# microsoft/protnote

Hardware: AMD Instinct MI355X
Metric: protein-label pairs/sec (fwd+bwd) (higher is better)
Workload: dtype f32

## Files before the change

### protnote_amd/csrc/abi_heads_eval.hpp

```cpp
extern "C" size_t pn_mlp_rows_ws_bytes(const pn_mlp* m, int rows) {
  size_t b = 0;
  int hmax = 0;
  for (int i = 0; i + 1 < m->nlayers; ++i) hmax = m->dims[i + 1] > hmax ? m->dims[i + 1] : hmax;
  b += 2 * al256((size_t)rows * hmax * sizeof(float));
  b += 2 * al256((size_t)hmax * sizeof(float));
  return b;
}

extern "C" int pn_mlp_rows_fwd_eval(const pn_mlp* m, const float* x, int ldx, int rows, float* y, void* ws,
                                    size_t ws_bytes, void* stream) {
  PN_OK(math_field_check(m->math_mode, "pn_mlp_rows_fwd_eval"));
  MathScope math_scope(m->math_mode);
  hipStream_t st = (hipStream_t)stream;
  if (m->nlayers < 1 || m->nlayers > PN_MAX_LAYERS) return fail("mlp: bad layer count %d", m->nlayers);
  for (int i = 0; i <= m->nlayers; ++i)
    if (i < m->nlayers && m->dims[i] % 4 != 0) return fail("mlp: dims[%d]=%d not a multiple of 4", i, m->dims[i]);
  if (ldx % 4 != 0) return fail("mlp: ldx %% 4 != 0");
  int hmax = 0;
  for (int i = 0; i + 1 < m->nlayers; ++i) hmax = m->dims[i + 1] > hmax ? m->dims[i + 1] : hmax;
  Bump bp(ws, ws_bytes);
  float* buf[2];
  buf[0] = bp.take<float>((size_t)rows * hmax);
  buf[1] = bp.take<float>((size_t)rows * hmax);
  float* s = bp.take<float>(hmax);
// ... 439 lines not shown
    if (part == nullptr) return fail("gemm_tn: no partial buffer");
    p.Cpart = part;
    p.ldc = p.N;
    long rps = (p.R + ns - 1) / ns;
    p.rows_per_split = (rps + 31) / 32 * 32;
    ns = (int)((p.R + p.rows_per_split - 1) / p.rows_per_split);
  }
  const unsigned tiles = (unsigned)((p.M / 256) * (p.N / 256));
  dim3 grid(tiles, (unsigned)ns);
  p.task_ns = 0;
  int* sync_ws = p.task_sync;
  p.task_sync = nullptr;
  if (p.M == 3072 && p.N == 3072 && ns >= 2) {
    p.task_ns = ns;
    grid = dim3(tn_task_grid(ns), 1);
    if (SYNC && sync_ws != nullptr && ns * 4 * 4 <= TN_SYNC_INTS) {
      HIP_OK(hipMemsetAsync(sync_ws, 0, (size_t)ns * 4 * 4 * sizeof(int), st));
      p.task_sync = sync_ws;
    }
  }
  {
    ProfScope ps(100 + TA_PLAIN * 10 + TB, 2.0 * (double)R_all * (double)p.M * (double)p.N, st);
    hipLaunchKernelGGL(kern, grid, dim3(512), TN_FAST_LDS_BYTES, st, p);
    if (tail != 0) {
      auto tk = gemm_tn_kernel<TA_PLAIN, TB, false>;
      static bool tattr[64] = {false};
      if (dev < 64 && !tattr[dev]) {
        HIP_OK(hipFuncSetAttribute((const void*)tk, hipFuncAttributeMaxDynamicSharedMemorySize, TN_LDS_BYTES));
        tattr[dev] = true;
      }
      TnParams t = p;
      t.R = R_all; t.row_base = R_all - tail; t.rows_per_split = 32;
      t.Cpart = part + (size_t)ns * p.M * p.N; t.ldc = p.N; t.task_ns = 0; t.task_sync = nullptr;
      hipLaunchKernelGGL(tk, dim3((unsigned)((p.M / 128) * (p.N / 128)), 1), dim3(256), TN_LDS_BYTES, st, t);
    }
  }
  HIP_OK(hipGetLastError());
  if (ns > 1 || tail != 0) {
    hipLaunchKernelGGL(k_splitk_reduce, dim3(nblk((long)p.M * p.N, 256)), dim3(256), 0, st, (const float*)part,
                       ns + (tail != 0 ? 1 : 0), p.M, p.N, (long)p.N, dst, ldd);
    HIP_OK(hipGetLastError());
  }
  return 0;
}

template <int TB, int NP = 3, bool TR = false, bool ABF16 = false>
static int launch_tn_bf16x3(TnParams p, float* dst, long ldd, float* part, size_t part_cap_floats, hipStream_t st) {
  void (*kern)(TnParams) = nullptr;
  constexpr bool SYNC = TR && TB == TB_AFFINE_RELU;
  void (*kern_alt)(TnParams) = nullptr;
  if constexpr (TR) {
    kern = gemm_tn_bf16tr_kernel<TB, ABF16, SYNC, true>;
    kern_alt = gemm_tn_bf16tr_kernel<TB, ABF16, SYNC, false>;
  } else {
    kern = gemm_tn_bf16x3_kernel<TB, NP>;
  }
  constexpr int LDS = TR ? TN_BF16TR_LDS_BYTES : 2 * 512 * 36 * (int)sizeof(float);
  static std::atomic<bool> attr_done[64];
  int dev = 0;
  HIP_OK(hipGetDevice(&dev));
  if (dev < 64 && !attr_done[dev]) {
    HIP_OK(hipFuncSetAttribute((const void*)kern, hipFuncAttributeMaxDynamicSharedMemorySize, LDS));
    if (kern_alt != nullptr) HIP_OK(hipFuncSetAttribute((const void*)kern_alt, hipFuncAttributeMaxDynamicSharedMemorySize, LDS));
    attr_done[dev] = true;
  }
  if (kern_alt != nullptr && !g_bf16_m16.load()) kern = kern_alt;
  int ns = tn_pick_split(p.R, p.M, p.N, part_cap_floats, 256, 1);
  if (ns == 1) {
    p.Cpart = dst;
    p.ldc = ldd;
    p.rows_per_split = (p.R + 31) / 32 * 32;
  } else {
    if (part == nullptr) return fail("gemm_tn: no partial buffer");
    p.Cpart = part;
    p.ldc = p.N;
    long rps = (p.R + ns - 1) / ns;
    p.rows_per_split = (rps + 31) / 32 * 32;
    ns = (int)((p.R + p.rows_per_split - 1) / p.rows_per_split);
  }
  const unsigned tiles = (unsigned)((p.M / 256) * (p.N / 256));
  dim3 grid(tiles, (unsigned)ns);
  p.task_ns = 0;
  int* sync_ws = p.task_sync;
  p.task_sync = nullptr;
  if (p.M == 3072 && p.N == 3072 && ns >= 2) {
    p.task_ns = ns;
    grid = dim3(tn_task_grid(ns), 1);
    if (SYNC && sync_ws != nullptr && ns * 4 * 4 <= TN_SYNC_INTS) {
      HIP_OK(hipMemsetAsync(sync_ws, 0, (size_t)ns * 4 * 4 * sizeof(int), st));
      p.task_sync = sync_ws;
    }
  }
  {
    ProfScope ps((NP == 3 ? 1100 : 1600) + TB, 2.0 * (double)p.R * (double)p.M * (double)p.N, st);
    hipLaunchKernelGGL(kern, grid, dim3(512), LDS, st, p);
  }
  HIP_OK(hipGetLastError());
  if (ns > 1) {
    hipLaunchKernelGGL(k_splitk_reduce, dim3(nblk((long)p.M * p.N, 256)), dim3(256), 0, st, (const float*)part, ns,
                       p.M, p.N, (long)p.N, dst, ldd);
    HIP_OK(hipGetLastError());
  }
  return 0;
}

template <int TA, int TB>
// ... 72 lines not shown
```

### protnote_amd/csrc/gemm_bf16x3.hpp

```cpp
#pragma once
#include "gemm_engine.hpp"
#include "gemm_tn.hpp"

#ifndef PN_B3_VALU
#define PN_B3_VALU 4
#endif

namespace pn {

typedef __bf16 bf16x4 __attribute__((ext_vector_type(4)));
typedef __bf16 bf16x8 __attribute__((ext_vector_type(8)));
typedef float f32x4 __attribute__((ext_vector_type(4)));

struct HiLo {
  bf16x4 hi, lo;
};

typedef __bf16 bf16x2 __attribute__((ext_vector_type(2)));
typedef float f32x2 __attribute__((ext_vector_type(2)));

__device__ __forceinline__ void split2(float x0, float x1, uint32_t& hi, uint32_t& lo) {
  const f32x2 x = {x0, x1};
  const bf16x2 h = __builtin_convertvector(x, bf16x2);
  hi = __builtin_bit_cast(uint32_t, h);
  const float r0 = x0 - __uint_as_float(hi << 16);
  const float r1 = x1 - __uint_as_float(hi & 0xffff0000u);
  const f32x2 r = {r0, r1};
  lo = __builtin_bit_cast(uint32_t, __builtin_convertvector(r, bf16x2));
}

__device__ __forceinline__ HiLo split4(float4 v) {
  uint32_t h0, l0, h1, l1;
  split2(v.x, v.y, h0, l0);
  split2(v.z, v.w, h1, l1);
  typedef uint32_t u32x2 __attribute__((ext_vector_type(2)));
  HiLo r;
  r.hi = __builtin_bit_cast(bf16x4, (u32x2){h0, h1});
  r.lo = __builtin_bit_cast(bf16x4, (u32x2){l0, l1});
  return r;
}

__device__ __forceinline__ bf16x8 round8(float4 v0, float4 v1) {
  typedef float f32x8 __attribute__((ext_vector_type(8)));
  const f32x8 x = {v0.x, v0.y, v0.z, v0.w, v1.x, v1.y, v1.z, v1.w};
  return __builtin_convertvector(x, bf16x8);
}

template <int AK, int EK, int WAVES_M, int WAVES_N, int WM, int WN, bool GEN = false, bool BDMA = false, int NP = 3>
__global__ __launch_bounds__(WAVES_M* WAVES_N * 64, (WAVES_M * WAVES_N) / 4) void gemm_nt_bf16x3_kernel(const GemmParams p) {
  static_assert(!BDMA || (!GEN && WAVES_M * WAVES_N == 8 && WAVES_N * WN * 32 == 256), "BDMA: 256-column pair-grid tiles");
  static_assert(NP == 3 || (NP == 1 && BDMA), "the single-product variant is built for the DMA-staged pair-grid kernel");
  constexpr int BK = 32;
  constexpr int NT = WAVES_M * WAVES_N * 64;
  constexpr int BM = WAVES_M * WM * 32;
  constexpr int BN = WAVES_N * WN * 32;
  constexpr int LDK = BK + 4;
  constexpr int KV = BK / 8;
  constexpr int RPP = NT / KV;
  constexpr int NQA = BM / RPP;
  constexpr int NQB = (BN + RPP - 1) / RPP;
  static_assert(BM % RPP == 0, "tile/thread mismatch");
  static_assert(AK == A_PLAIN || AK == A_AFFINE_RELU || AK == A_PAIRSUM_RELU || AK == A_CONV,
                "operand kind not built for bf16x3");
  static_assert(AK != A_CONV || GEN, "the conv gather needs the general path");
  constexpr int BPLANE = BN * 16;
  constexpr int STAGE = BDMA ? BM * LDK + 2 * BPLANE : (BM + BN) * LDK;

  extern __shared__ __attribute__((aligned(16))) float smem[];

  const int tid = threadIdx.x;
  const int lane = tid & 63;
  const int wave = tid >> 6;
  const int wm = wave / WAVES_N;
  const int wn = wave % WAVES_N;

  int tile_m, tile_n;
  if (!tile_coords<BM, BN>(p, tile_m, tile_n)) return;
  const int row0 = tile_m * BM;
  const int col0 = tile_n * BN;

  constexpr int NDQ = NP == 3 ? 4 : 2;
  const uint16_t* bsrc[4] = {nullptr, nullptr, nullptr, nullptr};
  unsigned bdst[4] = {0, 0, 0, 0};
  if constexpr (BDMA) {
    const int w = __builtin_amdgcn_readfirstlane(wave);
#pragma unroll
    for (int q = 0; q < NDQ; ++q) {
      const int c = NDQ * w + q;
      const int r = 16 * (c & 15) + (lane >> 2);
      const int g = (lane & 3) ^ ((r >> 2) & 3);
      bsrc[q] = ((c >> 4) ? p.w_lo : p.w_hi) + (long)(col0 + r) * p.Kseg + 8 * g;
      bdst[q] = (unsigned)(BM * LDK + (c >> 4) * BPLANE + 16 * (c & 15) * 16) * 4u;
    }
  }
  const unsigned lds0_b = (unsigned)(uintptr_t)(const __attribute__((address_space(3))) float*)smem;
  auto issue_b_dma = [&](int s_, int buf) {
#pragma unroll
    for (int q = 0; q < NDQ; ++q)
      tn_glds16(reinterpret_cast<const float*>(bsrc[q] + s_ * BK),
                __builtin_amdgcn_readfirstlane(lds0_b + (unsigned)(buf * STAGE) * 4u + bdst[q]));
  };

// ... 56 lines not shown
        for (int h = 0; h < 2; ++h) {
          rsc[h] = ld4(p.a_scale + c + 4 * kv + 16 * h);
          rsh[h] = ld4(p.a_shift + c + 4 * kv + 16 * h);
        }
      }
    } else {
      const int seg = s / spt;
      const int c0 = (s - seg * spt) * BK;
      bool kok[2];
      int cc[2];
#pragma unroll
      for (int h = 0; h < 2; ++h) {
        kok[h] = c0 + 4 * kv + 16 * h < p.Kseg;
        cc[h] = kok[h] ? c0 + 16 * h : -4 * kv;
      }
      avalid = 0;
      if constexpr (AK == A_CONV) {
        const int sh = (seg - p.nseg / 2) * p.dil;
#pragma unroll
        for (int q = 0; q < NQA; ++q) {
          const int tt = a_t[q] + sh;
          const bool ok = (a_t[q] < a_len[q]) && (tt >= 0) && (tt < a_len[q]);
#pragma unroll
          for (int h = 0; h < 2; ++h) {
            ra[q][h] = ld4(arow[q] + (long)(ok ? sh : 0) * p.lda + cc[h]);
            avalid |= ((ok && kok[h]) ? 1u : 0u) << (2 * q + h);
          }
        }
      } else {
#pragma unroll
        for (int q = 0; q < NQA; ++q)
#pragma unroll
          for (int h = 0; h < 2; ++h) {
            ra[q][h] = ld4(arow[q] + cc[h]);
            if constexpr (AK == A_PAIRSUM_RELU) ra2[q][h] = ld4(arow2[q] + cc[h]);
            avalid |= (kok[h] ? 1u : 0u) << (2 * q + h);
          }
      }
      if (AK == A_AFFINE_RELU || conv_affine) {
#pragma unroll
        for (int h = 0; h < 2; ++h) {
          rsc[h] = ld4(p.a_scale + 4 * kv + cc[h]);
          rsh[h] = ld4(p.a_shift + 4 * kv + cc[h]);
        }
      }
    }
  };
  auto fetch_b = [&](int s) {
    if constexpr (!GEN) {
      const int c = s * BK;
#pragma unroll
      for (int q = 0; q < NQB; ++q)
#pragma unroll
        for (int h = 0; h < 2; ++h) rb[q][h] = ld4(brow[q] + c + 16 * h);
    } else {
      const int seg = s / spt;
      const int c0 = (s - seg * spt) * BK;
      bmask = 0;
#pragma unroll
      for (int h = 0; h < 2; ++h) {
        const bool kok = c0 + 4 * kv + 16 * h < p.Kseg;
        const int cc = kok ? c0 + 16 * h : -4 * kv;
#pragma unroll
        for (int q = 0; q < NQB; ++q) {
          rb[q][h] = ld4(brow[q] + (long)seg * p.Kseg + cc);
          bmask |= ((kok && bvalid[q]) ? 1u : 0u) << (2 * q + h);
        }
      }
    }
  };
  auto pin_a = [&]() {
#pragma unroll
    for (int q = 0; q < NQA; ++q)
#pragma unroll
      for (int h = 0; h < 2; ++h) {
        pin4(ra[q][h]);
        if constexpr (AK == A_PAIRSUM_RELU) pin4(ra2[q][h]);
      }
  };
  auto pin_b = [&]() {
#pragma unroll
    for (int q = 0; q < NQB; ++q)
#pragma unroll
      for (int h = 0; h < 2; ++h) pin4(rb[q][h]);
  };

  auto store8 = [](float* dst, float4 v0, float4 v1) {
    if constexpr (NP == 1) {
      *reinterpret_cast<bf16x8*>(dst) = round8(v0, v1);
      return;
    }
    const HiLo a = split4(v0), b = split4(v1);
    bf16x8 hi, lo;
#pragma unroll
    for (int e = 0; e < 4; ++e) {
      hi[e] = a.hi[e];
      hi[4 + e] = b.hi[e];
      lo[e] = a.lo[e];
      lo[4 + e] = b.lo[e];
    }
    *reinterpret_cast<bf16x8*>(dst) = hi;
    *reinterpret_cast<bf16x8*>(dst + 4) = lo;
  };

  auto sel4 = [](bool ok, float4 v) {
    return make_float4(ok ? v.x : 0.f, ok ? v.y : 0.f, ok ? v.z : 0.f, ok ? v.w : 0.f);
  };
  auto commit_a = [&](int buf) {
    float* As = smem + buf * STAGE;
#pragma unroll
    for (int q = 0; q < NQA; ++q) {
      float4 v[2];
#pragma unroll
      for (int h = 0; h < 2; ++h) {
        v[h] = ra[q][h];
        if (AK == A_AFFINE_RELU || (AK == A_CONV && conv_affine)) {
          v[h].x = relu(fmaf(v[h].x, rsc[h].x, rsh[h].x));
          v[h].y = relu(fmaf(v[h].y, rsc[h].y, rsh[h].y));
          v[h].z = relu(fmaf(v[h].z, rsc[h].z, rsh[h].z));
          v[h].w = relu(fmaf(v[h].w, rsc[h].w, rsh[h].w));
        } else if constexpr (AK == A_PAIRSUM_RELU) {
          v[h].x = relu(v[h].x + ra2[q][h].x);
          v[h].y = relu(v[h].y + ra2[q][h].y);
          v[h].z = relu(v[h].z + ra2[q][h].z);
          v[h].w = relu(v[h].w + ra2[q][h].w);
        }
        if constexpr (GEN) v[h] = sel4((avalid >> (2 * q + h)) & 1u, v[h]);
      }
      store8(As + (r_in + q * RPP) * LDK + 8 * kv, v[0], v[1]);
    }
  };
  auto commit_b = [&](int buf) {
    float* Bs = smem + buf * STAGE + BM * LDK;
#pragma unroll
    for (int q = 0; q < NQB; ++q) {
      float4 v0 = rb[q][0], v1 = rb[q][1];
      if constexpr (GEN) {
        v0 = sel4((bmask >> (2 * q)) & 1u, v0);
        v1 = sel4((bmask >> (2 * q + 1)) & 1u, v1);
      }
      if (BN % RPP == 0 || r_in + q * RPP < BN) store8(Bs + (r_in + q * RPP) * LDK + 8 * kv, v0, v1);
    }
  };

  f32x16 acc[WM][WN];
#pragma unroll
  for (int i = 0; i < WM; ++i)
#pragma unroll
    for (int j = 0; j < WN; ++j)
#pragma unroll
      for (int e = 0; e < 16; ++e) acc[i][j][e] = 0.f;

  const int frag_row = lane & 31;
  const int frag_g = lane >> 5;

  auto compute = [&](int buf, auto ks_c) {
    constexpr int KS = decltype(ks_c)::value;
    const float* As = smem + buf * STAGE + (wm * WM * 32 + frag_row) * LDK + (2 * KS + frag_g) * 8;
    bf16x8 ah[WM], al[WM], bh[WN], bl[WN];
#pragma unroll
    for (int i = 0; i < WM; ++i) {
      ah[i] = *reinterpret_cast<const bf16x8*>(As + i * 32 * LDK);
      if constexpr (NP == 3) al[i] = *reinterpret_cast<const bf16x8*>(As + i * 32 * LDK + 4);
    }
    if constexpr (BDMA) {
      const float* Bs = smem + buf * STAGE + BM * LDK + (wn * WN * 32 + frag_row) * 16 +
                        4 * ((2 * KS + frag_g) ^ ((frag_row >> 2) & 3));
#pragma unroll
      for (int j = 0; j < WN; ++j) {
        bh[j] = *reinterpret_cast<const bf16x8*>(Bs + j * 32 * 16);
        if constexpr (NP == 3) bl[j] = *reinterpret_cast<const bf16x8*>(Bs + j * 32 * 16 + BPLANE);
      }
    } else {
      const float* Bs = smem + buf * STAGE + BM * LDK + (wn * WN * 32 + frag_row) * LDK + (2 * KS + frag_g) * 8;
#pragma unroll
      for (int j = 0; j < WN; ++j) {
        bh[j] = *reinterpret_cast<const bf16x8*>(Bs + j * 32 * LDK);
        bl[j] = *reinterpret_cast<const bf16x8*>(Bs + j * 32 * LDK + 4);
      }
    }
#pragma unroll
    for (int i = 0; i < WM; ++i)
#pragma unroll
      for (int j = 0; j < WN; ++j) {
        if constexpr (NP == 3) {
          acc[i][j] = __builtin_amdgcn_mfma_f32_32x32x16_bf16(al[i], bh[j], acc[i][j], 0, 0, 0);
          acc[i][j] = __builtin_amdgcn_mfma_f32_32x32x16_bf16(ah[i], bl[j], acc[i][j], 0, 0, 0);
        }
        acc[i][j] = __builtin_amdgcn_mfma_f32_32x32x16_bf16(ah[i], bh[j], acc[i][j], 0, 0, 0);
      }
  };

  using std::integral_constant;
  auto weave = [&](auto nvalu_c) {
    constexpr int NV = decltype(nvalu_c)::value;
    if constexpr (NP == 1) {
      __builtin_amdgcn_sched_group_barrier(0x100, WM + WN, 0);
#pragma unroll
      for (int i = 0; i < WM * WN; ++i) {
        __builtin_amdgcn_sched_group_barrier(0x008, 1, 0);
        __builtin_amdgcn_sched_group_barrier(0x002, NV, 0);
        if (i % 4 == 3) __builtin_amdgcn_sched_group_barrier(0x200, 1, 0);
      }
      return;
    }
    __builtin_amdgcn_sched_group_barrier(0x100, 2 * (WM + WN), 0);
#pragma unroll
    for (int i = 0; i < WM * WN * 3; ++i) {
      __builtin_amdgcn_sched_group_barrier(0x008, 1, 0);
      __builtin_amdgcn_sched_group_barrier(0x002, NV, 0);
      if (i % 3 == 2) __builtin_amdgcn_sched_group_barrier(0x200, 1, 0);
    }
  };
  if constexpr (BDMA) {
    issue_b_dma(0, 0);
    fetch_a(0);
    pin_a();
    commit_a(0);
    fetch_a(nslab > 1 ? 1 : 0);
    asm volatile("s_waitcnt vmcnt(0) lgkmcnt(0)" ::: "memory");
    __builtin_amdgcn_s_barrier();
    for (int s = 0; s + 1 < nslab; ++s) {
      const int cur = s & 1;
      const int nxt = s + 2 < nslab ? s + 2 : s + 1;
      __builtin_amdgcn_sched_barrier(0);
      pin_a();
      issue_b_dma(s + 1, cur ^ 1);
      __builtin_amdgcn_sched_barrier(0);
      compute(cur, integral_constant<int, 0>{});
      commit_a(cur ^ 1);
      weave(integral_constant<int, (AK == A_PLAIN ? PN_B3_VALU : PN_B3_VALU + 1)>{});
      __builtin_amdgcn_sched_barrier(0);
      asm volatile("s_waitcnt vmcnt(0)" ::: "memory");
      fetch_a(nxt);
      __builtin_amdgcn_sched_barrier(0);
      compute(cur, integral_constant<int, 1>{});
      __builtin_amdgcn_sched_barrier(0);
      asm volatile("s_waitcnt lgkmcnt(0)" ::: "memory");
      __builtin_amdgcn_s_barrier();
    }
    compute((nslab - 1) & 1, integral_constant<int, 0>{});
    __builtin_amdgcn_sched_barrier(0);
    compute((nslab - 1) & 1, integral_constant<int, 1>{});
    __syncthreads();
  } else {
  fetch_a(0);
  fetch_b(0);
  pin_a();
  pin_b();
  commit_a(0);
  commit_b(0);
  fetch_a(nslab > 1 ? 1 : 0);
  fetch_b(nslab > 1 ? 1 : 0);
  __syncthreads();
  for (int s = 0; s + 1 < nslab; ++s) {
    const int cur = s & 1;
    const int nxt = s + 2 < nslab ? s + 2 : s + 1;
    __builtin_amdgcn_sched_barrier(0);
    pin_a();
    compute(cur, integral_constant<int, 0>{});
    commit_a(cur ^ 1);
    weave(integral_constant<int, (AK == A_PLAIN ? PN_B3_VALU : PN_B3_VALU + 1)>{});
    __builtin_amdgcn_sched_barrier(0);
    fetch_a(nxt);
    __builtin_amdgcn_sched_barrier(0);
    pin_b();
    compute(cur, integral_constant<int, 1>{});
    commit_b(cur ^ 1);
    weave(integral_constant<int, PN_B3_VALU>{});
    __builtin_amdgcn_sched_barrier(0);
    fetch_b(nxt);
    __syncthreads();
  }
  compute((nslab - 1) & 1, integral_constant<int, 0>{});
  __builtin_amdgcn_sched_barrier(0);
  compute((nslab - 1) & 1, integral_constant<int, 1>{});
  __syncthreads();
  }

  gemm_epilogue<EK, WAVES_M, WAVES_N, WM, WN>(p, acc, row0, col0, tile_n, smem);
}

template <int TB, int NP = 3>
__global__ __launch_bounds__(512, PN_MINW) void gemm_tn_bf16x3_kernel(const TnParams p) {
  constexpr int BM = 256, BN = 256, BK = 32, LDK = BK + 4;
  constexpr int WM = 2, WN = 4;
  constexpr int STAGE = (BM + BN) * LDK;
  static_assert(TB == TB_PLAIN || TB == TB_AFFINE_RELU || TB == TB_PAIRSUM_RELU, "operand kind not built for bf16x3");

  extern __shared__ __attribute__((aligned(16))) float smem[];

  const int tid = threadIdx.x;
  const int lane = tid & 63;
  const int wave = tid >> 6;
  const int wm = wave >> 1, wn = wave & 1;

  const int ntn = p.N / BN, ntm = p.M / BM;
  int tile_m, tile_n;
  int split = blockIdx.y;
  if (p.task_ns > 0) {
    if (!tn_task_coords(p.task_ns, tile_m, tile_n, split)) return;
  } else if (PN_XCD && TB == TB_PAIRSUM_RELU && (ntm % 4 == 0) && (ntn % 2 == 0)) {
    const int rm = ntm / 4, rn = ntn / 2;
    const int xcd = blockIdx.x & 7, w = blockIdx.x >> 3;
    tile_m = (xcd >> 1) * rm + w / rn;
    tile_n = (xcd & 1) * rn + w % rn;
  } else if (PN_XCD && (ntm % 2 == 0) && (ntn % 4 == 0)) {
    const int rm = ntm / 2, rn = ntn / 4;
    const int xcd = blockIdx.x & 7, w = blockIdx.x >> 3;
    tile_m = (xcd >> 2) * rm + w / rn;
    tile_n = (xcd & 3) * rn + w % rn;
  } else {
    tile_n = blockIdx.x % ntn;
    tile_m = blockIdx.x / ntn;
  }
  const int m0 = tile_m * BM, n0 = tile_n * BN;
  const long r_begin = (long)split * p.rows_per_split;
  long r_end = r_begin + p.rows_per_split;
  if (r_end > p.R) r_end = p.R;

  const int col = tid & 255;
  const int kg = __builtin_amdgcn_readfirstlane(tid >> 8);
  float bs = 0.f, bt = 0.f;
  if constexpr (TB == TB_AFFINE_RELU) {
    bs = p.b_s[n0 + col];
    bt = p.b_t[n0 + col];
  }

  float ra[2][8], rb[2][8], rb2[2];
  const unsigned pB = (unsigned)p.pairB;
  const long lda = p.lda, ldb = p.ldb;

  auto fetch_a = [&](long k0, auto safe_c) {
    constexpr bool SAFE = decltype(safe_c)::value;
    const float* Ak = p.A + k0 * lda + m0;
    const int lim = (int)(r_end - 1 - k0);
#pragma unroll
// ... 56 lines not shown
      if constexpr (TB == TB_PAIRSUM_RELU) asm volatile("" : "+v"(rb2[g]));
    }
  };

  auto store8 = [](float* dst, const float (&v)[8]) {
    if constexpr (NP == 1) {
      *reinterpret_cast<bf16x8*>(dst) = round8(make_float4(v[0], v[1], v[2], v[3]), make_float4(v[4], v[5], v[6], v[7]));
      return;
    }
    const HiLo a = split4(make_float4(v[0], v[1], v[2], v[3])), b = split4(make_float4(v[4], v[5], v[6], v[7]));
    bf16x8 hi, lo;
#pragma unroll
    for (int e = 0; e < 4; ++e) {
      hi[e] = a.hi[e];
      hi[4 + e] = b.hi[e];
      lo[e] = a.lo[e];
      lo[4 + e] = b.lo[e];
    }
    *reinterpret_cast<bf16x8*>(dst) = hi;
    *reinterpret_cast<bf16x8*>(dst + 4) = lo;
  };

  auto commit_a = [&](int buf, long k0, auto safe_c) {
    constexpr bool SAFE = decltype(safe_c)::value;
    float* As = smem + buf * STAGE;
#pragma unroll
    for (int g = 0; g < 2; ++g) {
      float a[8];
#pragma unroll
      for (int e = 0; e < 8; ++e) {
        a[e] = ra[g][e];
        if (SAFE && k0 + 8 * (kg + 2 * g) + e >= r_end) a[e] = 0.f;
      }
      store8(As + col * LDK + 8 * (kg + 2 * g), a);
    }
  };
  auto commit_b = [&](int buf, long k0, auto safe_c) {
    constexpr bool SAFE = decltype(safe_c)::value;
    float* Bs = smem + buf * STAGE + BM * LDK;
#pragma unroll
    for (int g = 0; g < 2; ++g) {
      float b[8];
#pragma unroll
      for (int e = 0; e < 8; ++e) {
        b[e] = rb[g][e];
        if constexpr (TB == TB_AFFINE_RELU) b[e] = relu(fmaf(b[e], bs, bt));
        if constexpr (TB == TB_PAIRSUM_RELU) b[e] = relu(b[e] + rb2[g]);
        if (SAFE && k0 + 8 * (kg + 2 * g) + e >= r_end) b[e] = 0.f;
      }
      store8(Bs + col * LDK + 8 * (kg + 2 * g), b);
    }
  };

  f32x16 acc[WM][WN];
#pragma unroll
  for (int i = 0; i < WM; ++i)
#pragma unroll
    for (int j = 0; j < WN; ++j)
#pragma unroll
      for (int e = 0; e < 16; ++e) acc[i][j][e] = 0.f;

  const int frag_row = lane & 31;
  const int frag_g = lane >> 5;
  auto compute = [&](int buf, auto ks_c) {
    constexpr int KS = decltype(ks_c)::value;
    const float* As = smem + buf * STAGE + (wm * WM * 32 + frag_row) * LDK + (2 * KS + frag_g) * 8;
    const float* Bs = smem + buf * STAGE + BM * LDK + (wn * WN * 32 + frag_row) * LDK + (2 * KS + frag_g) * 8;
    bf16x8 ah[WM], al[WM], bh[WN], bl[WN];
#pragma unroll
    for (int i = 0; i < WM; ++i) {
      ah[i] = *reinterpret_cast<const bf16x8*>(As + i * 32 * LDK);
      if constexpr (NP == 3) al[i] = *reinterpret_cast<const bf16x8*>(As + i * 32 * LDK + 4);
    }
#pragma unroll
    for (int j = 0; j < WN; ++j) {
      bh[j] = *reinterpret_cast<const bf16x8*>(Bs + j * 32 * LDK);
      if constexpr (NP == 3) bl[j] = *reinterpret_cast<const bf16x8*>(Bs + j * 32 * LDK + 4);
    }
#pragma unroll
    for (int i = 0; i < WM; ++i)
#pragma unroll
      for (int j = 0; j < WN; ++j) {
        if constexpr (NP == 3) {
          acc[i][j] = __builtin_amdgcn_mfma_f32_32x32x16_bf16(al[i], bh[j], acc[i][j], 0, 0, 0);
          acc[i][j] = __builtin_amdgcn_mfma_f32_32x32x16_bf16(ah[i], bl[j], acc[i][j], 0, 0, 0);
        }
        acc[i][j] = __builtin_amdgcn_mfma_f32_32x32x16_bf16(ah[i], bh[j], acc[i][j], 0, 0, 0);
      }
  };

  using std::integral_constant;
  using std::false_type;
  using std::true_type;
  auto weave = [&](auto nvalu_c) {
    constexpr int NV = decltype(nvalu_c)::value;
    if constexpr (NP == 1) {
      __builtin_amdgcn_sched_group_barrier(0x100, WM + WN, 0);
#pragma unroll
      for (int i = 0; i < WM * WN; ++i) {
        __builtin_amdgcn_sched_group_barrier(0x008, 1, 0);
        __builtin_amdgcn_sched_group_barrier(0x002, 3 * NV, 0);
        if (i % 4 == 3) __builtin_amdgcn_sched_group_barrier(0x200, 1, 0);
      }
      return;
    }
    __builtin_amdgcn_sched_group_barrier(0x100, 2 * (WM + WN), 0);
#pragma unroll
    for (int i = 0; i < WM * WN * 3; ++i) {
      __builtin_amdgcn_sched_group_barrier(0x008, 1, 0);
      __builtin_amdgcn_sched_group_barrier(0x002, NV, 0);
      if (i % 3 == 2) __builtin_amdgcn_sched_group_barrier(0x200, 1, 0);
    }
  };
  if (r_begin < r_end) {
    const long span = r_end - r_begin;
    const int nf = (int)(span / BK);
    const int ns = nf + ((span % BK) ? 1 : 0);
    auto K0 = [&](int t) { return r_begin + (long)t * BK; };
    auto body = [&](int t, auto safe_c) {
      const int cur = t & 1;
      const int t2 = t + 2 < ns ? t + 2 : t + 1;
      __builtin_amdgcn_sched_barrier(0);
      pin_a();
      compute(cur, integral_constant<int, 0>{});
      commit_a(cur ^ 1, K0(t + 1), safe_c);
      weave(integral_constant<int, 2>{});
      __builtin_amdgcn_sched_barrier(0);
      fetch_a(K0(t2), safe_c);
      __builtin_amdgcn_sched_barrier(0);
      pin_b();
      compute(cur, integral_constant<int, 1>{});
      commit_b(cur ^ 1, K0(t + 1), safe_c);
      weave(integral_constant<int, (TB == TB_PLAIN ? 2 : 3)>{});
      __builtin_amdgcn_sched_barrier(0);
      fetch_b(K0(t2), safe_c);
      __syncthreads();
    };
    fetch_a(K0(0), true_type{});
    fetch_b(K0(0), true_type{});
    pin_a();
    pin_b();
    commit_a(0, K0(0), true_type{});
    commit_b(0, K0(0), true_type{});
    fetch_a(K0(ns > 1 ? 1 : 0), true_type{});
    fetch_b(K0(ns > 1 ? 1 : 0), true_type{});
    __syncthreads();
    int t = 0;
    for (; t + 2 < nf; ++t) body(t, false_type{});
    for (; t + 1 < ns; ++t) body(t, true_type{});
    compute((ns - 1) & 1, integral_constant<int, 0>{});
    __builtin_amdgcn_sched_barrier(0);
    compute((ns - 1) & 1, integral_constant<int, 1>{});
  }

  float* out = p.Cpart + (long)split * p.M * p.ldc;
  const int hl = lane >> 5, cl = lane & 31;
#pragma unroll
  for (int i = 0; i < WM; ++i)
#pragma unroll
    for (int j = 0; j < WN; ++j) {
      const int n = n0 + (wn * WN + j) * 32 + cl;
#pragma unroll
      for (int e = 0; e < 16; ++e) {
        const int m = m0 + (wm * WM + i) * 32 + (e & 3) + 8 * (e >> 2) + 4 * hl;
        out[(long)m * p.ldc + n] = acc[i][j][e];
      }
    }
}

__global__ void k_split_planes(const float* __restrict__ W, long ldw, int N, int K, uint16_t* __restrict__ hi,
                               uint16_t* __restrict__ lo) {
  const long i = ((long)blockIdx.x * blockDim.x + threadIdx.x) * 4;
  if (i >= (long)N * K) return;
  const long n = i / K;
  const int pos = (int)(i - n * K);
  const int blk = pos >> 5, in = pos & 31, g = in >> 3, half = (in >> 2) & 1;
  const HiLo s = split4(ld4(W + n * ldw + blk * 32 + half * 16 + 4 * g));
  *reinterpret_cast<bf16x4*>(hi + i) = s.hi;
  *reinterpret_cast<bf16x4*>(lo + i) = s.lo;
}

}
```

### protnote_amd/csrc/protnote_hip.hip

```cpp
#include <hip/hip_runtime.h>
#include <stdarg.h>
#include <stdio.h>
#include <stdlib.h>
#include <string.h>

#include "../../include/protnote_hip.h"
#include "common.hpp"
#include "gemm_engine.hpp"
#include "gemm_bf16x3.hpp"
#include "gemm_bf16.hpp"
#include "gemm_dma.hpp"
#include "gemm_conv_dma.hpp"
#include "gemm_conv_f64.hpp"
#include "gemm_tn_fast.hpp"
#include "train_kernels.hpp"
#include "bwd_bf16_dz.hpp"
#include "fwd_bf16_h.hpp"
#include "gemm_bf16_m16.hpp"

using namespace pn;

static thread_local char g_err[512] = "";

static int fail(const char* fmt, ...) {
// ... 302 lines not shown
  return 0;
}

static std::atomic<int> g_bwd_math{0};
extern "C" int pn_set_backward_math(int mode) {
  if (mode != 0 && mode != 1) return fail("pn_set_backward_math: 0 (as the forward) or 1 (bf16, one product)");
  g_bwd_math = mode;
  return 0;
}
extern "C" int pn_get_backward_math(void) { return g_bwd_math; }
static thread_local bool tl_bwd_bf16 = false;
static thread_local bool tl_dz_bf16 = false;
struct BwdBf16Scope {
  bool prev;
  explicit BwdBf16Scope(bool on) : prev(tl_bwd_bf16) { tl_bwd_bf16 = on; }
  ~BwdBf16Scope() {
    tl_bwd_bf16 = prev;
    tl_dz_bf16 = false;
  }
};

static std::atomic<int> g_fwd_math{0};
extern "C" int pn_set_forward_math(int mode) {
  if (mode != 0 && mode != 1) return fail("pn_set_forward_math: 0 (as math_mode) or 1 (bf16, one product)");
  g_fwd_math = mode;
  return 0;
}
extern "C" int pn_get_forward_math(void) { return g_fwd_math; }
static thread_local bool tl_fwd_bf16 = false;
struct FwdBf16Scope {
  bool prev;
  explicit FwdBf16Scope(bool on) : prev(tl_fwd_bf16) { tl_fwd_bf16 = on; }
  ~FwdBf16Scope() { tl_fwd_bf16 = prev; }
};
static bool fwd_bf16_requested(const pn_pairhead* hd) {
  const int m = hd->forward_math == 0 ? g_fwd_math.load(std::memory_order_relaxed) : hd->forward_math - 1;
  return m == 1 && hd->dropout_p == 0.f;
}
static int fwd_math_of(const pn_pairhead* hd, bool* bf16) {
  if (hd->forward_math < 0 || hd->forward_math > 2)
    return fail("pairhead: forward_math %d (0 = library default, 1 = as math_mode, 2 = bf16)", hd->forward_math);
  const int m = hd->forward_math == 0 ? g_fwd_math.load(std::memory_order_relaxed) : hd->forward_math - 1;
  *bf16 = (m == 1) && hd->dropout_p == 0.f;
  return 0;
}

static std::atomic<int> g_b3_dma{1};
static bool use_b3_dma() { return g_b3_dma == 1; }
extern "C" int pn_set_b3_dma(int on) {
  g_b3_dma = on ? 1 : 0;
  return 0;
}

template <int AK, int EK, int WAVES_N, int WN, bool GEN, bool BDMA = false, int NP = 3>
static int launch_gemm_bf16x3(const GemmParams& p, hipStream_t st) {
  using Cfg = GemmCfg<4, WAVES_N, 2, WN, 32>;
  if constexpr (!GEN && !BDMA && WAVES_N * WN * 32 == 256) {
    if (p.wsplit != nullptr && use_b3_dma() && p.Nstore == p.N)
      return launch_gemm_bf16x3<AK, EK, WAVES_N, WN, GEN, true>(p, st);
  }
  auto kern = gemm_nt_bf16x3_kernel<AK, EK, 4, WAVES_N, 2, WN, GEN, BDMA, NP>;
  constexpr int LDS_BYTES = BDMA ? 2 * (256 * 36 + 2 * 256 * 16) * (int)sizeof(float) : Cfg::LDS_BYTES;
  static std::atomic<bool> attr_done[64];
  int dev = 0;
  HIP_OK(hipGetDevice(&dev));
  if (dev < 64 && !attr_done[dev]) {
    HIP_OK(hipFuncSetAttribute((const void*)kern, hipFuncAttributeMaxDynamicSharedMemorySize, LDS_BYTES));
    attr_done[dev] = true;
  }
  if (p.M <= 0 || p.Nstore <= 0) return 0;
  if (p.Kseg % 4 != 0) return fail("gemm: K segment %d not a multiple of 4", p.Kseg);
  const long tm = (p.M + Cfg::BM - 1) / Cfg::BM;
  const long tn = (p.Nstore + Cfg::BN - 1) / Cfg::BN;
  GemmParams pp = p;
  pp.xcd_bc = (PN_XCD && tm >= 16) ? ((tn % 8 == 0) ? 8 : ((tn % 4 == 0) ? 4 : 0)) : 0;
  if (!GEN && AK == A_PAIRSUM_RELU && pp.xcd_bc && tm >= 64) pp.xcd_bc = 1;
  pp.xcd_br = pp.xcd_bc ? 32 / pp.xcd_bc : 0;
  long grid = tm * tn;
  if (pp.xcd_bc) {
    const long nblk = ((tm + pp.xcd_br - 1) / pp.xcd_br) * (tn / pp.xcd_bc);
    grid = ((nblk + 7) / 8) * 8 * 32;
  }
  if (grid > 0x7fffffffL) return fail("gemm: grid too large");
  if constexpr (BDMA) {
    pp.w_hi = p.wsplit;
    pp.w_lo = p.wsplit + (size_t)p.N * p.Kseg;
    hipLaunchKernelGGL(k_split_planes, dim3(nblk((long)p.N * p.Kseg / 4, 256)), dim3(256), 0, st, p.W, p.ldw, p.N, p.Kseg,
                       p.wsplit, p.wsplit + (size_t)p.N * p.Kseg);
  }
  {
    ProfScope ps((NP == 3 ? 1000 : 1500) + AK * 10 + EK, 2.0 * (double)p.M * (double)p.N * (double)p.nseg * (double)p.Kseg, st);
    hipLaunchKernelGGL(kern, dim3((unsigned)grid), dim3(Cfg::NT), LDS_BYTES, st, pp);
  }
  HIP_OK(hipGetLastError());
  return finish_col_stats(p, tm, st);
}

static std::atomic<int> g_bwd_deep{7};
extern "C" int pn_set_bwd_deep(int mask) {
  g_bwd_deep = mask & 7;
  return 0;
}
static int launch_gemm_bf16_single(const GemmParams& p, hipStream_t st) {
  auto kern = gemm_nt_bf16_kernel<E_STORE>;
  static std::atomic<bool> attr_done[64];
  int dev = 0;
  HIP_OK(hipGetDevice(&dev));
  if (dev < 64 && !attr_done[dev]) {
    HIP_OK(hipFuncSetAttribute((const void*)kern, hipFuncAttributeMaxDynamicSharedMemorySize, NT_BF16_LDS_BYTES));
    attr_done[dev] = true;
  }
  if (p.M <= 0 || p.Nstore <= 0) return 0;
  const long tm = (p.M + 255) / 256, tn = p.N / 256;
  GemmParams pp = p;
  pp.xcd_bc = (PN_XCD && tm >= 16) ? ((tn % 8 == 0) ? 8 : ((tn % 4 == 0) ? 4 : 0)) : 0;
  pp.xcd_br = pp.xcd_bc ? 32 / pp.xcd_bc : 0;
  long grid = tm * tn;
  if (pp.xcd_bc) {
    const long nblk_ = ((tm + pp.xcd_br - 1) / pp.xcd_br) * (tn / pp.xcd_bc);
    grid = ((nblk_ + 7) / 8) * 8 * 32;
  }
  if (grid > 0x7fffffffL) return fail("gemm: grid too large");
  pp.w_hi = p.wsplit;
  pp.w_lo = p.wsplit + (size_t)p.N * p.Kseg;
  hipLaunchKernelGGL(k_split_planes, dim3(nblk((long)p.N * p.Kseg / 4, 256)), dim3(256), 0, st, p.W, p.ldw, p.N, p.Kseg,
                     p.wsplit, p.wsplit + (size_t)p.N * p.Kseg);
  {
    ProfScope ps(1500 + A_PLAIN * 10 + E_STORE, 2.0 * (double)p.M * (double)p.N * (double)p.Kseg, st);
    hipLaunchKernelGGL(kern, dim3((unsigned)grid), dim3(512), NT_BF16_LDS_BYTES, st, pp);
  }
  HIP_OK(hipGetLastError());
  return 0;
}

static std::atomic<int> g_bf16_m16{1};
extern "C" int pn_set_bf16_mfma16(int on) {
  g_bf16_m16 = on ? 1 : 0;
  return 0;
}
template <int EK>
static int bf16dma_kernel(void (**out)(GemmParams)) {
  static std::atomic<bool> attr_done[64];
  int dev = 0;
  HIP_OK(hipGetDevice(&dev));
  if (dev < 64 && !attr_done[dev]) {
    HIP_OK(hipFuncSetAttribute((const void*)gemm_nt_bf16dma_kernel<EK>, hipFuncAttributeMaxDynamicSharedMemorySize, NT_BF16DMA_LDS_BYTES));
    HIP_OK(hipFuncSetAttribute((const void*)gemm_nt_bf16m16_kernel<EK>, hipFuncAttributeMaxDynamicSharedMemorySize, NT_BF16DMA_LDS_BYTES));
    attr_done[dev] = true;
  }
  *out = g_bf16_m16.load() ? gemm_nt_bf16m16_kernel<EK> : gemm_nt_bf16dma_kernel<EK>;
  return 0;
}

static int launch_gemm_bf16dma(const GemmParams& p, hipStream_t st) {
  void (*kern)(GemmParams) = nullptr;
  if (int rc = bf16dma_kernel<E_STORE>(&kern)) return rc;
  if (p.M <= 0 || p.Nstore <= 0) return 0;
  if (p.wsplit == nullptr || p.Kseg % 64 != 0 || p.N % 256 != 0 || p.Nstore != p.N || (long)256 * p.lda * 4 >= (1L << 32) ||
      (long)256 * p.Kseg * 2 >= (1L << 32))
    return fail("gemm (bf16 dz): shape %d x %d x %d not supported", p.M, p.N, p.Kseg);
  const long tm = (p.M + 255) / 256, tn = p.N / 256;
  GemmParams pp = p;
  pp.xcd_bc = (PN_XCD && tm >= 16) ? ((tn % 8 == 0) ? 8 : ((tn % 4 == 0) ? 4 : 0)) : 0;
  pp.xcd_br = pp.xcd_bc ? 32 / pp.xcd_bc : 0;
  long grid = tm * tn;
  if (pp.xcd_bc) {
    const long nblk_ = ((tm + pp.xcd_br - 1) / pp.xcd_br) * (tn / pp.xcd_bc);
    grid = ((nblk_ + 7) / 8) * 8 * 32;
  }
  if (grid > 0x7fffffffL) return fail("gemm: grid too large");
  pp.w_hi = p.wsplit;
  hipLaunchKernelGGL(k_round_plane, dim3(nblk((long)p.N * p.Kseg / 4, 256)), dim3(256), 0, st, p.W, p.ldw, p.N, p.Kseg, p.wsplit);
  {
    ProfScope ps(1500 + A_PLAIN * 10 + E_STORE, 2.0 * (double)p.M * (double)p.N * (double)p.Kseg, st);
    hipLaunchKernelGGL(kern, dim3((unsigned)grid), dim3(512), NT_BF16DMA_LDS_BYTES, st, pp);
  }
  HIP_OK(hipGetLastError());
  return 0;
}

#ifndef PN_BIG
#define PN_BIG 1
#endif
static std::atomic<int> g_fwd_staged{1};
extern "C" int pn_set_fwd_staged(int on) {
  g_fwd_staged = on ? 1 : 0;
  return 0;
}
static thread_local bool tl_fwd_nostage = false;
static const long FWD_H_ROWS = 262144;
static bool fwd_staged_shape(int h) { return PN_BIG && h % 256 == 0 && h >= 256 && h <= 8192; }
static bool fwd_staged_on(bool fwd_bf16, int h) { return fwd_bf16 && g_fwd_staged == 1 && !tl_fwd_nostage && fwd_staged_shape(h); }
// ... 447 lines not shown
```

Before: 1.253 million.

## Use 16x16x32 bf16 MFMA fragments in the bf16x3 NT and TN GEMM kernels

Adds an M16 variant of the three-product bf16x3 split GEMM kernels (NT pair-grid and TN weight-gradient) that tiles each wave's output as 16x16 fragments and issues mfma_f32_16x16x32_bf16 instead of the 32x32 path. It includes new LDS fragment addressing, a reworked instruction-interleave schedule, a new epilogue and output store, and a B-row load based on a single base pointer. The variant is on by default through the existing bf16_m16 flag, which is moved earlier so the bf16x3 launchers can read it. The goal is higher MFMA throughput and a better fit for K=32 steps, at the cost of more accumulator fragments and more LDS reads.

Result: no change. 1.253 million (median of 2 runs) (-0.0%).

```diff
diff --git a/protnote_amd/csrc/abi_heads_eval.hpp b/protnote_amd/csrc/abi_heads_eval.hpp
--- a/protnote_amd/csrc/abi_heads_eval.hpp
+++ b/protnote_amd/csrc/abi_heads_eval.hpp
@@ -515,6 +515,9 @@
   if constexpr (TR) {
     kern = gemm_tn_bf16tr_kernel<TB, ABF16, SYNC, true>;
     kern_alt = gemm_tn_bf16tr_kernel<TB, ABF16, SYNC, false>;
+  } else if constexpr (NP == 3) {
+    kern = gemm_tn_bf16x3_kernel<TB, NP, true>;
+    kern_alt = gemm_tn_bf16x3_kernel<TB, NP>;
   } else {
     kern = gemm_tn_bf16x3_kernel<TB, NP>;
   }
diff --git a/protnote_amd/csrc/gemm_bf16x3.hpp b/protnote_amd/csrc/gemm_bf16x3.hpp
--- a/protnote_amd/csrc/gemm_bf16x3.hpp
+++ b/protnote_amd/csrc/gemm_bf16x3.hpp
@@ -46,8 +46,12 @@
   return __builtin_convertvector(x, bf16x8);
 }
 
-template <int AK, int EK, int WAVES_M, int WAVES_N, int WM, int WN, bool GEN = false, bool BDMA = false, int NP = 3>
+template <int EK, int WAVES_M, int WAVES_N, int FM, int FN>
+__device__ __forceinline__ void gemm_epilogue_m16(const GemmParams& p, f32x4 (&acc)[FM][FN], int row0, int col0, int tile_n, float* smem);
+
+template <int AK, int EK, int WAVES_M, int WAVES_N, int WM, int WN, bool GEN = false, bool BDMA = false, int NP = 3, bool M16 = false>
 __global__ __launch_bounds__(WAVES_M* WAVES_N * 64, (WAVES_M * WAVES_N) / 4) void gemm_nt_bf16x3_kernel(const GemmParams p) {
+  static_assert(!M16 || (NP == 3 && !GEN && WN % 2 == 0 && (EK == E_STORE || EK == E_ROWDOT)), "M16: the three-product pair-grid kernels");
   static_assert(!BDMA || (!GEN && WAVES_M * WAVES_N == 8 && WAVES_N * WN * 32 == 256), "BDMA: 256-column pair-grid tiles");
   static_assert(NP == 3 || (NP == 1 && BDMA), "the single-product variant is built for the DMA-staged pair-grid kernel");
   constexpr int BK = 32;
@@ -210,7 +214,10 @@
 #pragma unroll
       for (int q = 0; q < NQB; ++q)
 #pragma unroll
-        for (int h = 0; h < 2; ++h) rb[q][h] = ld4(brow[q] + c + 16 * h);
+        for (int h = 0; h < 2; ++h) {
+          if constexpr (M16) rb[q][h] = ld4(brow[0] + (long)q * RPP * p.ldw + c + 16 * h);
+          else rb[q][h] = ld4(brow[q] + c + 16 * h);
+        }
     } else {
       const int seg = s / spt;
       const int c0 = (s - seg * spt) * BK;
@@ -301,19 +308,68 @@
     }
   };
 
-  f32x16 acc[WM][WN];
-#pragma unroll
-  for (int i = 0; i < WM; ++i)
-#pragma unroll
-    for (int j = 0; j < WN; ++j)
-#pragma unroll
-      for (int e = 0; e < 16; ++e) acc[i][j][e] = 0.f;
-
-  const int frag_row = lane & 31;
-  const int frag_g = lane >> 5;
-
+  constexpr int FM = 2 * WM, FN = 2 * WN, FH = FN / 2;
+  f32x16 acc[M16 ? 1 : WM][M16 ? 1 : WN];
+  f32x4 acc16[M16 ? FM : 1][M16 ? FN : 1];
+  if constexpr (M16) {
+#pragma unroll
+    for (int i = 0; i < FM; ++i)
+#pragma unroll
+      for (int j = 0; j < FN; ++j)
+#pragma unroll
+        for (int e = 0; e < 4; ++e) acc16[i][j][e] = 0.f;
+  } else {
+#pragma unroll
+    for (int i = 0; i < WM; ++i)
+#pragma unroll
+      for (int j = 0; j < WN; ++j)
+#pragma unroll
+        for (int e = 0; e < 16; ++e) acc[i][j][e] = 0.f;
+  }
+
+  const int frag_row = M16 ? (lane & 15) : (lane & 31);
+  const int frag_g = M16 ? (lane >> 4) : (lane >> 5);
+
+  bf16x8 fah[M16 ? FM : 1], fal[M16 ? FM : 1];
   auto compute = [&](int buf, auto ks_c) {
     constexpr int KS = decltype(ks_c)::value;
+    if constexpr (M16) {
+      if constexpr (KS == 0 || !BDMA) {
+        const float* As = smem + buf * STAGE + (wm * FM * 16 + frag_row) * LDK + frag_g * 8;
+#pragma unroll
+        for (int i = 0; i < FM; ++i) {
+          fah[i] = *reinterpret_cast<const bf16x8*>(As + i * 16 * LDK);
+          fal[i] = *reinterpret_cast<const bf16x8*>(As + i * 16 * LDK + 4);
+        }
+      }
+      bf16x8 bh[FH], bl[FH];
+      if constexpr (BDMA) {
+        const float* Bs = smem + buf * STAGE + BM * LDK + ((wn * FN + KS * FH) * 16 + frag_row) * 16 +
+                          4 * (frag_g ^ ((frag_row >> 2) & 3));
+#pragma unroll
+        for (int j = 0; j < FH; ++j) {
+          bh[j] = *reinterpret_cast<const bf16x8*>(Bs + j * 16 * 16);
+          bl[j] = *reinterpret_cast<const bf16x8*>(Bs + j * 16 * 16 + BPLANE);
+        }
+      } else {
+        const float* Bs = smem + buf * STAGE + BM * LDK + ((wn * FN + KS * FH) * 16 + frag_row) * LDK + frag_g * 8;
+#pragma unroll
+        for (int j = 0; j < FH; ++j) {
+          bh[j] = *reinterpret_cast<const bf16x8*>(Bs + j * 16 * LDK);
+          bl[j] = *reinterpret_cast<const bf16x8*>(Bs + j * 16 * LDK + 4);
+        }
+      }
+#pragma unroll
+      for (int j = 0; j < FH; ++j)
+#pragma unroll
+        for (int i = 0; i < FM; ++i) {
+          f32x4& c = acc16[i][KS * FH + j];
+          c = __builtin_amdgcn_mfma_f32_16x16x32_bf16(fal[i], bh[j], c, 0, 0, 0);
+          c = __builtin_amdgcn_mfma_f32_16x16x32_bf16(fah[i], bl[j], c, 0, 0, 0);
+          c = __builtin_amdgcn_mfma_f32_16x16x32_bf16(fah[i], bh[j], c, 0, 0, 0);
+        }
+      return;
+    }
     const float* As = smem + buf * STAGE + (wm * WM * 32 + frag_row) * LDK + (2 * KS + frag_g) * 8;
     bf16x8 ah[WM], al[WM], bh[WN], bl[WN];
 #pragma unroll
@@ -350,7 +406,7 @@
   };
 
   using std::integral_constant;
-  auto weave = [&](auto nvalu_c) {
+  auto weave = [&](auto nvalu_c, auto region_c) {
     constexpr int NV = decltype(nvalu_c)::value;
     if constexpr (NP == 1) {
       __builtin_amdgcn_sched_group_barrier(0x100, WM + WN, 0);
@@ -359,6 +415,23 @@
         __builtin_amdgcn_sched_group_barrier(0x008, 1, 0);
         __builtin_amdgcn_sched_group_barrier(0x002, NV, 0);
         if (i % 4 == 3) __builtin_amdgcn_sched_group_barrier(0x200, 1, 0);
+      }
+      return;
+    }
+    if constexpr (M16) {
+      constexpr int RG = decltype(region_c)::value;
+      __builtin_amdgcn_sched_group_barrier(0x100, (RG == 0 || !BDMA ? 2 * FM : 0) + 2, 0);
+#pragma unroll
+      for (int j = 0; j < FH; ++j) {
+        if (j + 1 < FH) __builtin_amdgcn_sched_group_barrier(0x100, 2, 0);
+#pragma unroll
+        for (int m = 0; m < FM * 3 / 2; ++m) {
+          __builtin_amdgcn_sched_group_barrier(0x008, 1, 0);
+          if constexpr (NV / 2 > 0) __builtin_amdgcn_sched_group_barrier(0x002, NV / 2, 0);
+          __builtin_amdgcn_sched_group_barrier(0x008, 1, 0);
+          if constexpr (NV - NV / 2 > 0) __builtin_amdgcn_sched_group_barrier(0x002, NV - NV / 2, 0);
+          if (NV > 0 && m % 3 == 2) __builtin_amdgcn_sched_group_barrier(0x200, 1, 0);
+        }
       }
       return;
     }
@@ -387,12 +460,13 @@
       __builtin_amdgcn_sched_barrier(0);
       compute(cur, integral_constant<int, 0>{});
       commit_a(cur ^ 1);
-      weave(integral_constant<int, (AK == A_PLAIN ? PN_B3_VALU : PN_B3_VALU + 1)>{});
+      weave(integral_constant<int, (AK == A_PLAIN ? PN_B3_VALU : PN_B3_VALU + 1)>{}, integral_constant<int, 0>{});
       __builtin_amdgcn_sched_barrier(0);
       asm volatile("s_waitcnt vmcnt(0)" ::: "memory");
       fetch_a(nxt);
       __builtin_amdgcn_sched_barrier(0);
       compute(cur, integral_constant<int, 1>{});
+      if constexpr (M16) weave(integral_constant<int, 0>{}, integral_constant<int, 1>{});
       __builtin_amdgcn_sched_barrier(0);
       asm volatile("s_waitcnt lgkmcnt(0)" ::: "memory");
       __builtin_amdgcn_s_barrier();
@@ -418,14 +492,14 @@
     pin_a();
     compute(cur, integral_constant<int, 0>{});
     commit_a(cur ^ 1);
-    weave(integral_constant<int, (AK == A_PLAIN ? PN_B3_VALU : PN_B3_VALU + 1)>{});
+    weave(integral_constant<int, (AK == A_PLAIN ? PN_B3_VALU : PN_B3_VALU + 1)>{}, integral_constant<int, 0>{});
     __builtin_amdgcn_sched_barrier(0);
     fetch_a(nxt);
     __builtin_amdgcn_sched_barrier(0);
     pin_b();
     compute(cur, integral_constant<int, 1>{});
     commit_b(cur ^ 1);
-    weave(integral_constant<int, PN_B3_VALU>{});
+    weave(integral_constant<int, PN_B3_VALU>{}, integral_constant<int, 1>{});
     __builtin_amdgcn_sched_barrier(0);
     fetch_b(nxt);
     __syncthreads();
@@ -436,11 +510,13 @@
   __syncthreads();
   }
 
-  gemm_epilogue<EK, WAVES_M, WAVES_N, WM, WN>(p, acc, row0, col0, tile_n, smem);
+  if constexpr (M16) gemm_epilogue_m16<EK, WAVES_M, WAVES_N, FM, FN>(p, acc16, row0, col0, tile_n, smem);
+  else gemm_epilogue<EK, WAVES_M, WAVES_N, WM, WN>(p, acc, row0, col0, tile_n, smem);
 }
 
-template <int TB, int NP = 3>
+template <int TB, int NP = 3, bool M16 = false>
 __global__ __launch_bounds__(512, PN_MINW) void gemm_tn_bf16x3_kernel(const TnParams p) {
+  static_assert(!M16 || NP == 3, "M16: the three-product kernel");
   constexpr int BM = 256, BN = 256, BK = 32, LDK = BK + 4;
   constexpr int WM = 2, WN = 4;
   constexpr int STAGE = (BM + BN) * LDK;
@@ -603,18 +679,57 @@
     }
   };
 
-  f32x16 acc[WM][WN];
-#pragma unroll
-  for (int i = 0; i < WM; ++i)
-#pragma unroll
-    for (int j = 0; j < WN; ++j)
-#pragma unroll
-      for (int e = 0; e < 16; ++e) acc[i][j][e] = 0.f;
-
-  const int frag_row = lane & 31;
-  const int frag_g = lane >> 5;
+  constexpr int FM = 2 * WM, FN = 2 * WN, FH = FN / 2;
+  f32x16 acc[M16 ? 1 : WM][M16 ? 1 : WN];
+  f32x4 acc16[M16 ? FM : 1][M16 ? FN : 1];
+  if constexpr (M16) {
+#pragma unroll
+    for (int i = 0; i < FM; ++i)
+#pragma unroll
+      for (int j = 0; j < FN; ++j)
+#pragma unroll
+        for (int e = 0; e < 4; ++e) acc16[i][j][e] = 0.f;
+  } else {
+#pragma unroll
+    for (int i = 0; i < WM; ++i)
+#pragma unroll
+      for (int j = 0; j < WN; ++j)
+#pragma unroll
+        for (int e = 0; e < 16; ++e) acc[i][j][e] = 0.f;
+  }
+
+  const int frag_row = M16 ? (lane & 15) : (lane & 31);
+  const int frag_g = M16 ? (lane >> 4) : (lane >> 5);
+  bf16x8 fah[M16 ? FM : 1], fal[M16 ? FM : 1];
   auto compute = [&](int buf, auto ks_c) {
     constexpr int KS = decltype(ks_c)::value;
+    if constexpr (M16) {
+      if constexpr (KS == 0) {
+        const float* As = smem + buf * STAGE + (wm * FM * 16 + frag_row) * LDK + frag_g * 8;
+#pragma unroll
+        for (int i = 0; i < FM; ++i) {
+          fah[i] = *reinterpret_cast<const bf16x8*>(As + i * 16 * LDK);
+          fal[i] = *reinterpret_cast<const bf16x8*>(As + i * 16 * LDK + 4);
+        }
+      }
+      const float* Bs = smem + buf * STAGE + BM * LDK + ((wn * FN + KS * FH) * 16 + frag_row) * LDK + frag_g * 8;
+      bf16x8 bh[FH], bl[FH];
+#pragma unroll
+      for (int j = 0; j < FH; ++j) {
+        bh[j] = *reinterpret_cast<const bf16x8*>(Bs + j * 16 * LDK);
+        bl[j] = *reinterpret_cast<const bf16x8*>(Bs + j * 16 * LDK + 4);
+      }
+#pragma unroll
+      for (int j = 0; j < FH; ++j)
+#pragma unroll
+        for (int i = 0; i < FM; ++i) {
+          f32x4& c = acc16[i][KS * FH + j];
+          c = __builtin_amdgcn_mfma_f32_16x16x32_bf16(fal[i], bh[j], c, 0, 0, 0);
+          c = __builtin_amdgcn_mfma_f32_16x16x32_bf16(fah[i], bl[j], c, 0, 0, 0);
+          c = __builtin_amdgcn_mfma_f32_16x16x32_bf16(fah[i], bh[j], c, 0, 0, 0);
+        }
+      return;
+    }
     const float* As = smem + buf * STAGE + (wm * WM * 32 + frag_row) * LDK + (2 * KS + frag_g) * 8;
     const float* Bs = smem + buf * STAGE + BM * LDK + (wn * WN * 32 + frag_row) * LDK + (2 * KS + frag_g) * 8;
     bf16x8 ah[WM], al[WM], bh[WN], bl[WN];
@@ -643,7 +758,7 @@
   using std::integral_constant;
   using std::false_type;
   using std::true_type;
-  auto weave = [&](auto nvalu_c) {
+  auto weave = [&](auto nvalu_c, auto region_c) {
     constexpr int NV = decltype(nvalu_c)::value;
     if constexpr (NP == 1) {
       __builtin_amdgcn_sched_group_barrier(0x100, WM + WN, 0);
@@ -652,6 +767,23 @@
         __builtin_amdgcn_sched_group_barrier(0x008, 1, 0);
         __builtin_amdgcn_sched_group_barrier(0x002, 3 * NV, 0);
         if (i % 4 == 3) __builtin_amdgcn_sched_group_barrier(0x200, 1, 0);
+      }
+      return;
+    }
+    if constexpr (M16) {
+      constexpr int RG = decltype(region_c)::value;
+      __builtin_amdgcn_sched_group_barrier(0x100, (RG == 0 ? 2 * FM : 0) + 2, 0);
+#pragma unroll
+      for (int j = 0; j < FH; ++j) {
+        if (j + 1 < FH) __builtin_amdgcn_sched_group_barrier(0x100, 2, 0);
+#pragma unroll
+        for (int m = 0; m < FM * 3 / 2; ++m) {
+          __builtin_amdgcn_sched_group_barrier(0x008, 1, 0);
+          if constexpr (NV / 2 > 0) __builtin_amdgcn_sched_group_barrier(0x002, NV / 2, 0);
+          __builtin_amdgcn_sched_group_barrier(0x008, 1, 0);
+          if constexpr (NV - NV / 2 > 0) __builtin_amdgcn_sched_group_barrier(0x002, NV - NV / 2, 0);
+          if (NV > 0 && m % 3 == 2) __builtin_amdgcn_sched_group_barrier(0x200, 1, 0);
+        }
       }
       return;
     }
@@ -675,14 +807,14 @@
       pin_a();
       compute(cur, integral_constant<int, 0>{});
       commit_a(cur ^ 1, K0(t + 1), safe_c);
-      weave(integral_constant<int, 2>{});
+      weave(integral_constant<int, 2>{}, integral_constant<int, 0>{});
       __builtin_amdgcn_sched_barrier(0);
       fetch_a(K0(t2), safe_c);
       __builtin_amdgcn_sched_barrier(0);
       pin_b();
       compute(cur, integral_constant<int, 1>{});
       commit_b(cur ^ 1, K0(t + 1), safe_c);
-      weave(integral_constant<int, (TB == TB_PLAIN ? 2 : 3)>{});
+      weave(integral_constant<int, (TB == TB_PLAIN ? 2 : 3)>{}, integral_constant<int, 1>{});
       __builtin_amdgcn_sched_barrier(0);
       fetch_b(K0(t2), safe_c);
       __syncthreads();
@@ -705,6 +837,21 @@
   }
 
   float* out = p.Cpart + (long)split * p.M * p.ldc;
+  if constexpr (M16) {
+    const int rq = lane >> 4, c16 = lane & 15;
+#pragma unroll
+    for (int i = 0; i < FM; ++i)
+#pragma unroll
+      for (int j = 0; j < FN; ++j) {
+        const int n = n0 + (wn * FN + j) * 16 + c16;
+#pragma unroll
+        for (int e = 0; e < 4; ++e) {
+          const int m = m0 + (wm * FM + i) * 16 + 4 * rq + e;
+          out[(long)m * p.ldc + n] = acc16[i][j][e];
+        }
+      }
+    return;
+  }
   const int hl = lane >> 5, cl = lane & 31;
 #pragma unroll
   for (int i = 0; i < WM; ++i)
diff --git a/protnote_amd/csrc/protnote_hip.hip b/protnote_amd/csrc/protnote_hip.hip
--- a/protnote_amd/csrc/protnote_hip.hip
+++ b/protnote_amd/csrc/protnote_hip.hip
@@ -378,6 +378,12 @@
   return 0;
 }
 
+static std::atomic<int> g_bf16_m16{1};
+extern "C" int pn_set_bf16_mfma16(int on) {
+  g_bf16_m16 = on ? 1 : 0;
+  return 0;
+}
+
 template <int AK, int EK, int WAVES_N, int WN, bool GEN, bool BDMA = false, int NP = 3>
 static int launch_gemm_bf16x3(const GemmParams& p, hipStream_t st) {
   using Cfg = GemmCfg<4, WAVES_N, 2, WN, 32>;
@@ -385,15 +391,20 @@
     if (p.wsplit != nullptr && use_b3_dma() && p.Nstore == p.N)
       return launch_gemm_bf16x3<AK, EK, WAVES_N, WN, GEN, true>(p, st);
   }
-  auto kern = gemm_nt_bf16x3_kernel<AK, EK, 4, WAVES_N, 2, WN, GEN, BDMA, NP>;
+  void (*kern)(GemmParams) = gemm_nt_bf16x3_kernel<AK, EK, 4, WAVES_N, 2, WN, GEN, BDMA, NP>;
+  void (*kern16)(GemmParams) = nullptr;
+  if constexpr (NP == 3 && !GEN && (EK == E_STORE || EK == E_ROWDOT))
+    kern16 = gemm_nt_bf16x3_kernel<AK, EK, 4, WAVES_N, 2, WN, GEN, BDMA, NP, true>;
   constexpr int LDS_BYTES = BDMA ? 2 * (256 * 36 + 2 * 256 * 16) * (int)sizeof(float) : Cfg::LDS_BYTES;
   static std::atomic<bool> attr_done[64];
   int dev = 0;
   HIP_OK(hipGetDevice(&dev));
   if (dev < 64 && !attr_done[dev]) {
     HIP_OK(hipFuncSetAttribute((const void*)kern, hipFuncAttributeMaxDynamicSharedMemorySize, LDS_BYTES));
+    if (kern16 != nullptr) HIP_OK(hipFuncSetAttribute((const void*)kern16, hipFuncAttributeMaxDynamicSharedMemorySize, LDS_BYTES));
     attr_done[dev] = true;
   }
+  if (kern16 != nullptr && g_bf16_m16.load()) kern = kern16;
   if (p.M <= 0 || p.Nstore <= 0) return 0;
   if (p.Kseg % 4 != 0) return fail("gemm: K segment %d not a multiple of 4", p.Kseg);
   const long tm = (p.M + Cfg::BM - 1) / Cfg::BM;
@@ -459,11 +470,6 @@
   return 0;
 }
 
-static std::atomic<int> g_bf16_m16{1};
-extern "C" int pn_set_bf16_mfma16(int on) {
-  g_bf16_m16 = on ? 1 : 0;
-  return 0;
-}
 template <int EK>
 static int bf16dma_kernel(void (**out)(GemmParams)) {
   static std::atomic<bool> attr_done[64];
```
